# stripe/rainier

Hardware: AMD Instinct MI355X
Metric: leapfrog steps/sec (all chains) (higher is better)
Workload: dtype f64

## Files before the change

rainier_amd/csrc/device/rh_lane.hip.h:

```cpp
#if RH_NROWTARGETS > 0 && !RH_HAS_GATHER && !RH_BIGTH && !RH_BIGN && !RH_LK_LDS
#ifndef RH_LANE_W
#define RH_LANE_W 8
#endif
#ifndef RH_LANE_R
#define RH_LANE_R 8
#endif
#ifndef RH_LANE_C
#define RH_LANE_C 2
#endif
#ifndef RH_LANE_FEED_ROWS
#define RH_LANE_FEED_ROWS 0
#endif
typedef const double __attribute__((address_space(4))) *rh_ccol_t;
struct rh_lane_rows { const double *p[RH_NROWTARGETS]; };
constexpr bool rh_lane_rowfed(int nc) { return RH_LANE_FEED_ROWS && (nc == 1 || nc == 2 || nc == 4 || nc == 8); }
constexpr int rh_lane_set(int nc) { return 16 / nc < RH_LANE_R ? 16 / nc : RH_LANE_R; }
template <int S, int NC> RH_DEV void rh_lane_request(double (&c)[S][NC], rh_ccol_t rp, const long long row) {
#pragma unroll
  for (int u = 0; u < S; u++)
#pragma unroll
    for (int j = 0; j < NC; j++) c[u][j] = rp[(row + u) * NC + j];
}
template <int S, int NC> RH_DEV void rh_lane_arrived(const double (&c)[S][NC]) {
#pragma unroll
  for (int u = 0; u < S; u++)
#pragma unroll
    for (int j = 0; j < NC; j++) asm volatile("" ::"s"(c[u][j]));
}
template <int T, bool NV>
RH_DEV void rh_lane_targets(const double (&th)[RH_LANE_C][RH_NTH], const rh_model_data &d, const rh_lane_rows *rows, const int w, const int split, const int nsplit,
                            const int *__restrict__ lp, const int nvalid, const int chains, double *__restrict__ partial,
                            double *red, int &err) {
  if constexpr (T < RH_NTARGETS) {
    typedef rh_target<T> TG;
    if constexpr (TG::HAS_ROWS) {
      constexpr int NC = TG::NCOLS, R = RH_LANE_R, C = RH_LANE_C, W = RH_LANE_W;
      constexpr int NA = TG::NACC > 0 ? TG::NACC : 1;
      const int lane = threadIdx.x & 63;
      double inv[C][TG::NINV > 0 ? TG::NINV : 1];
#pragma unroll
      for (int k = 0; k < C; k++) TG::invariants(th[k], inv[k], err);
      const long long n = d.nrows[T];
      const long long blocks = (n + R - 1) / R, per = (blocks + nsplit - 1) / nsplit, perw = (per + W - 1) / W;
      long long s0 = (long long)split * per * R, s1 = s0 + per * R;
      if (s0 > n) s0 = n;
      if (s1 > n) s1 = n;
      long long r0 = s0 + (long long)w * perw * R, r1 = r0 + perw * R;
      if (r0 > s1) r0 = s1;
      if (r1 > s1) r1 = s1;
      rh_ccol_t cp[NC];
#pragma unroll
      for (int j = 0; j < NC; j++) cp[j] = (rh_ccol_t)d.cols[TG::COL0 + j];
      double acc[C][NA];
#pragma unroll
      for (int k = 0; k < C; k++)
#pragma unroll
        for (int o = 0; o < NA; o++) acc[k][o] = 0.0;
      long long kb = r0;
      if constexpr (rh_lane_rowfed(NC)) {
        constexpr int S = rh_lane_set(NC);
        static_assert(R % S == 0 && S * NC * 2 * 2 <= 64, "two sets of whole rows in 64 scalar registers, a block of R rows in whole sets");
        const rh_ccol_t rp = (rh_ccol_t)rows->p[TG::ROWT];
        const int nsets = (int)((r1 - kb) / S);
        const long long last = kb + (long long)(nsets > 0 ? nsets - 1 : 0) * S;
        auto rows_of = [&](const double (&cur)[S][NC]) {
#pragma unroll
          for (int u = 0; u < S; u++)
#pragma unroll
            for (int k = 0; k < C; k++) rh_row<TG, NV>(th[k], inv[k], cur[u], acc[k], err);
// ... 23 lines not shown
        double c[R][NC];
#pragma unroll
        for (int u = 0; u < R; u++)
#pragma unroll
          for (int j = 0; j < NC; j++) c[u][j] = cp[j][kb + u];
#pragma unroll
        for (int u = 0; u < R; u++)
#pragma unroll
          for (int k = 0; k < C; k++) rh_row<TG, NV>(th[k], inv[k], c[u], acc[k], err);
      }
      for (; kb < r1; kb++) {
        double c[NC];
#pragma unroll
        for (int j = 0; j < NC; j++) c[j] = cp[j][kb];
#pragma unroll
        for (int k = 0; k < C; k++) rh_row<TG, NV>(th[k], inv[k], c, acc[k], err);
      }
      }
#pragma unroll
      for (int k = 0; k < C; k++)
#pragma unroll
        for (int o = 0; o < NA; o++) red[((w * C + k) * NA + o) * 64 + lane] = acc[k][o];
      __syncthreads();
      for (int t = threadIdx.x; t < C * NA * 64; t += 64 * W) {
        const int ko = t >> 6, l = t & 63, k = ko / NA, o = ko - k * NA;
        double s = red[ko * 64 + l];
#pragma unroll
        for (int ww = 1; ww < W; ww++) s += red[(ww * C * NA + ko) * 64 + l];
        const int slot = k * 64 + l;
        if (slot < nvalid) partial[(((size_t)TG::ROWT * nsplit + split) * chains + lp[slot]) * RH_NACC_MAX + o] = s;
      }
      __syncthreads();
    }
    rh_lane_targets<T + 1, NV>(th, d, rows, w, split, nsplit, lp, nvalid, chains, partial, red, err);
  }
}
RH_DEV void rh_grad_lane_body(const rh_model_data &d, const rh_lane_rows *rows, const double *__restrict__ q, const int *__restrict__ list,
                              const int *__restrict__ nlive, const int *__restrict__ vflag, double *__restrict__ partial, int *__restrict__ err_out,
                              int *__restrict__ n_running, const int chains, const int nsplit, const int xcd_aware, double *red) {
  const int lane = threadIdx.x & 63, w = __builtin_amdgcn_readfirstlane((int)(threadIdx.x >> 6));
  const int b = blockIdx.x;
  if (b == 0 && threadIdx.x == 0) *n_running = 0;
  const int nl = rh_live_count(nlive, chains);
  int split, group;
  rh_grad_map(b, nsplit, xcd_aware, split, group);
  const int slot0 = group * (64 * RH_LANE_C);
  if (slot0 >= nl) return;
  double th[RH_LANE_C][RH_NTH];
  bool gonly = rh_any_value_only<0>::v && vflag != nullptr;
#pragma unroll
  for (int k = 0; k < RH_LANE_C; k++) {
    const int c = rh_live_chain(list, slot0 + k * 64 + lane, nl);
    if constexpr (rh_any_value_only<0>::v) gonly = gonly && vflag[c] == 2;
#pragma unroll
    for (int i = 0; i < RH_NVARS; i++) th[k][i] = q[(size_t)c * RH_NVARS + i];
  }
  int err = 0;
  if constexpr (rh_any_value_only<0>::v) {
    if (__all(gonly)) rh_lane_targets<0, false>(th, d, rows, w, split, nsplit, list + slot0, nl - slot0, chains, partial, red, err);
    else rh_lane_targets<0, true>(th, d, rows, w, split, nsplit, list + slot0, nl - slot0, chains, partial, red, err);
  } else
  rh_lane_targets<0, true>(th, d, rows, w, split, nsplit, list + slot0, nl - slot0, chains, partial, red, err);
  if (__any(err != 0) && lane == 0) atomicOr(err_out, 1);
}
#if !RH_LANE_FEED_ROWS
extern "C" __global__ void __launch_bounds__(64 * RH_LANE_W)
rh_grad_lane_kernel(const rh_model_data d, const double *__restrict__ q, const int *__restrict__ list, const int *__restrict__ nlive,
                    const int *__restrict__ vflag, double *__restrict__ partial, int *__restrict__ err_out, int *__restrict__ n_running,
                    const int chains, const int nsplit, const int xcd_aware) {
  __shared__ double red[RH_LANE_W * RH_LANE_C * RH_NACC_MAX * 64];
  rh_grad_lane_body(d, nullptr, q, list, nlive, vflag, partial, err_out, n_running, chains, nsplit, xcd_aware, red);
}
#else
extern "C" __global__ void __launch_bounds__(64 * RH_LANE_W)
rh_grad_lane_kernel(const rh_model_data d, const rh_lane_rows rows, const double *__restrict__ q, const int *__restrict__ list,
                    const int *__restrict__ nlive, const int *__restrict__ vflag, double *__restrict__ partial, int *__restrict__ err_out,
                    int *__restrict__ n_running, const int chains, const int nsplit, const int xcd_aware) {
  __shared__ double red[RH_LANE_W * RH_LANE_C * RH_NACC_MAX * 64];
  rh_grad_lane_body(d, &rows, q, list, nlive, vflag, partial, err_out, n_running, chains, nsplit, xcd_aware, red);
}
#endif
#endif
```

rainier_amd/csrc/engine.cpp:

```cpp
#include <hip/hip_runtime.h>
#include <hip/hiprtc.h>

#include <cmath>
#include <chrono>
#include <cstdio>
#include <cstdlib>
#include <cstring>
#include <algorithm>
#include <atomic>
#include <fstream>
#include <functional>
#include <map>
#include <memory>
#include <mutex>
#include <sstream>
#include <string>
#include <thread>
#include <vector>

#include <dlfcn.h>
#include <sys/stat.h>
#include <unistd.h>

#include "../../include/rainier_hip.h"
// ... 188 lines not shown
  bool pending = false, prev_rec = false;
  std::vector<int> livelog[2];
  std::vector<char> was_ticked[2];
};
struct RoundRec {
  bool open = false;
  int pool = 0;
  bool live[2] = {false, false};
  int B[2] = {0, 0};
};

struct rh_sampler {
  hipFunction_t k_chain = nullptr, k_tick = nullptr;
  int state_words = 0, dense_off = 0, pack_l = 64;
  int off_Pq = -1, off_Pg = -1, off_PU = -1;
  rh_model *m = nullptr;
  rh_cfg_dev cfg{};
  int chains = 0;
  void *d_state = nullptr, *d_seeds = nullptr, *d_mass = nullptr, *d_draws = nullptr, *d_stats = nullptr, *d_running = nullptr;
  int it_done = 0;
  bool started = false, warmed = false;
  hipEvent_t e0 = nullptr, e1 = nullptr;
  double kernel_ms = 0, total_ms = 0;
  int64_t chain_slots = 0, steady_launches = 0, steady_evals = 0;
  double steady_ms = 0;
  int64_t launches = 0;
  bool tick_engine = false;
  int nsplit = 0, xcd_aware = 1;
  bool compact = true;
  void *d_qbuf = nullptr, *d_active = nullptr;
  void *d_rec[2] = {nullptr, nullptr};
  bool fuse = false;
  bool lane_walk = false;
  bool lane_rows = false;
  std::vector<Lane> lanes;
  int round_cap = 0;
  int next_pool = 0;
  RoundRec round;
  std::vector<rh_chain_stats_dev> last_stats;
  int64_t grads_at_reset = 0;
};
int guard(rh_model *m, const std::function<void()> &fn) {
  try { fn(); return RH_OK; }
  catch (const Fail &f) { g_err = f.msg; if (m) m->err = f.msg; return f.code; }
  catch (const std::exception &e) { g_err = e.what(); if (m) m->err = e.what(); return RH_E_INVALID; }
}
DrawsView sampler_draws(rh_sampler *s) {
  return {s->d_draws, s->m->device, s->m->stream, s->chains, s->it_done, (int)s->m->prog.n_params, s->cfg.iterations, &s->m->mu, &s->m->err, s->m};
}

namespace {

void assemble_source(rh_model *m) {
  std::string defines, targets, err;
  if (const char *e = rh::knob("RH_GRAD_PIPELINE")) m->eopt.grad_pipeline = std::atoi(e);
  if (const char *e = rh::knob("RH_FMA_ADDS")) m->eopt.fma_adds = std::atoi(e) != 0;
  if (const char *e = rh::knob("RH_XFUSE")) m->eopt.xfuse = std::atoi(e) != 0;
  if (const char *e = rh::knob("RH_SIMPLIFY")) m->eopt.simplify = std::atoi(e) != 0;
  if (const char *e = rh::knob("RH_PACK")) m->eopt.pack = std::atoi(e) != 0;
  if (const char *e = rh::knob("RH_FAST_LOG")) m->eopt.fast_log = std::atoi(e) != 0;
  if (const char *e = rh::knob("RH_FORCE_BIGN")) m->eopt.force_bign = std::atoi(e) != 0;
  if (const char *e = rh::knob("RH_LOGIT_LINK")) m->eopt.logit_link = std::atoi(e) != 0;
  if (const char *e = rh::knob("RH_CONST_POOL")) m->eopt.const_pool = std::atoi(e) != 0;
  if (const char *e = rh::knob("RH_CHUNK")) if (m->eopt.chunk == 0) m->eopt.chunk = std::max(0, std::atoi(e));
  if (m->eopt.chunk > 0) {
    m->eopt.rows_unroll = 1; m->eopt.grad_unroll = 1; m->eopt.grad_pipeline = 0; m->unroll_auto = false;
    m->eopt.grad_chains = 1;
// ... 1219 lines not shown
        void *sb = nullptr;
        const size_t bytes = sizeof(double) * (size_t)chains * m->gather_count[rt];
        HIPCHK(hipMalloc(&sb, bytes));
        owned.push_back(sb);
        HIPCHK(hipMemset(sb, 0, bytes));
        gd.sbuf[rt] = (double *)sb;
      }
    }
    HIPCHK(hipDeviceSynchronize());
  }
  ~GatherBufs() { for (void *p : owned) (void)hipFree(p); }
};

int default_nsplit(const rh_model *m, int chains) {
  const int ngroups = (chains + m->grad_k - 1) / m->grad_k;
  int64_t max_rows = 1;
  for (size_t t = 0; t < m->prog.targets.size(); t++) if (m->prog.targets[t].n_cols) max_rows = std::max<int64_t>(max_rows, m->data.nrows[t]);
  int nsplit = (int)std::max<int64_t>(1, ((m->eopt.grad_pipeline == 2 ? 2048 : 4096) + ngroups - 1) / ngroups);
  if (m->info.gather_mode) nsplit = (int)std::max<int64_t>(1, (16384 + ngroups - 1) / ngroups);
  if (const char *e = rh::knob("RH_GATHER_WG")) if (m->info.gather_mode) nsplit = (int)std::max<int64_t>(1, (std::atoi(e) + ngroups - 1) / ngroups);
  if (m->k_grad_glm) { const int ctiles = (chains + 15) / 16; nsplit = (int)std::max<int64_t>(1, (2048 + ctiles - 1) / ctiles); }
  nsplit = ((nsplit + 7) / 8) * 8;
  const int64_t cap = std::max<int64_t>(8, (max_rows / 2048) / 8 * 8);
  return (int)std::min<int64_t>(nsplit, cap);
}

int64_t lane_max_rows(const rh_model *m) {
  int64_t max_rows = 1;
  for (size_t t = 0; t < m->prog.targets.size(); t++) if (m->prog.targets[t].n_cols) max_rows = std::max<int64_t>(max_rows, m->data.nrows[t]);
  return max_rows;
}
thread_local int g_total_chains = 0;
thread_local int g_shard_walk = -1;
bool walk_is_lane(rh_model *m, bool static_hmc, int total_chains) {
  if (g_shard_walk >= 0) return g_shard_walk == 1 && ensure_lane(m) != nullptr;
  int forced = 0;
  if (const char *e = rh::knob("RH_GRAD_WALK")) forced = std::strcmp(e, "tile") == 0 ? 1 : (std::strcmp(e, "lane") == 0 ? 2 : 0);
  if (!rh_plan::walk_is_lane(true, static_hmc, m->grad_chains_req, total_chains, lane_max_rows(m), forced)) return false;
  return ensure_lane(m) != nullptr;
}
int lane_nsplit(const rh_model *m, int total_chains) {
  return rh_plan::lane_nsplit(total_chains, lane_max_rows(m));
}
bool feed_is_rows(rh_model *m) {
  int forced = 0;
  if (const char *e = rh::knob("RH_LANE_FEED")) forced = std::strcmp(e, "cols") == 0 ? 1 : (std::strcmp(e, "rows") == 0 ? 2 : 0);
  if (!rh_plan::feed_is_rows(true, forced)) return false;
  if (!rh_plan::feed_is_rows(ensure_lane_rows(m) != nullptr, forced)) return false;
  std::vector<long long> want;
  for (size_t t = 0; t < m->prog.targets.size(); t++) if (m->prog.targets[t].n_cols) want.push_back(m->data.nrows[t]);
  return m->k_grad_lane_rows && rh_plan::lane_rows_cover((int)want.size(), want.data(), (int)m->dev_rows_n.size(), m->dev_rows_n.data(), m->dev_rows.data());
}

void launch_grad(rh_model *m, GatherBufs *gb, void *d_q, void *d_list, void *d_nlive, void *d_vflag, void *d_partial, void *d_graderr, void *d_running,
                 int chains, int nsplit, int xcd, hipStream_t stream = nullptr, bool lane_walk = false, bool lane_rows = false) {
  if (!stream) stream = m->stream;
  if (lane_walk) {
    const int lgroups = (chains + rh_plan::kLaneGroup - 1) / rh_plan::kLaneGroup;
    if (lane_rows) {
      void *ra[] = {&m->data, m->dev_rows.data(), &d_q, &d_list, &d_nlive, &d_vflag, &d_partial, &d_graderr, &d_running, &chains, &nsplit, &xcd};
      launch(m->k_grad_lane_rows, (unsigned)(lgroups * nsplit), 64 * rh_plan::kLaneW, stream, ra);
      return;
    }
    void *la[] = {&m->data, &d_q, &d_list, &d_nlive, &d_vflag, &d_partial, &d_graderr, &d_running, &chains, &nsplit, &xcd};
    launch(m->k_grad_lane, (unsigned)(lgroups * nsplit), 64 * rh_plan::kLaneW, stream, la);
    return;
  }
  const int ngroups = (chains + m->grad_k - 1) / m->grad_k;
  if (m->info.gather_mode) {
    void *ga[] = {&m->data, &gb->gd, &d_q, &d_list, &d_nlive, &d_vflag, &d_partial, &d_graderr, &d_running, &chains, &nsplit};
    if (gb->any_big) launch(m->k_grad_gather, (unsigned)(ngroups * nsplit), 64, stream, ga);
    if (gb->any_small) launch(m->k_grad_gather_scan, (unsigned)(ngroups * nsplit), 64, stream, ga);
    return;
  }
  void *args[] = {&m->data, &d_q, &d_list, &d_nlive, &d_vflag, &d_partial, &d_graderr, &d_running, &chains, &nsplit, &xcd};
  if (m->k_grad_glm) {
    const int ctiles = (chains + 15) / 16;
    const unsigned blocks = (unsigned)(((ctiles + m->glm_w - 1) / m->glm_w) * nsplit);
    const unsigned tile = (unsigned)m->glm_ncols * 66u * (unsigned)sizeof(double);
    const unsigned lds = (2u * tile + (m->lk_lds ? 6176u : 0u) <= 160u * 1024u ? 2u : 1u) * tile;
    HIPCHK(hipModuleLaunchKernel(m->k_grad_glm, blocks, 1, 1, 64u * m->glm_w, 1, 1, lds, stream, args, nullptr));
  } else
    launch(m->k_grad, (unsigned)(ngroups * nsplit), 64, stream, args);
}
}

extern "C" int rh_density_eval(rh_model *m, const double *q, int32_t chains, double *logp, double *grad) {
  return rh_density_eval_ex(m, q, chains, RH_ENGINE_AUTO, 0, logp, grad);
}

extern "C" int rh_density_eval_ex(rh_model *m, const double *q, int32_t chains, int32_t engine, int32_t grad_splits,
                                  double *logp, double *grad) {
  if (!m || !m->loaded) { g_err = "rh_density_eval: model not loaded"; return RH_E_INVALID; }
  if (!q || !logp || !grad || chains <= 0) { m->err = g_err = "rh_density_eval: bad arguments"; return RH_E_INVALID; }
  if (engine < RH_ENGINE_AUTO || engine > RH_ENGINE_TICK || grad_splits < 0 || grad_splits > 65536) { m->err = g_err = "rh_density_eval_ex: unknown engine / bad grad_splits"; return RH_E_INVALID; }
  if (engine == RH_ENGINE_TICK && m->n_row_targets == 0) { m->err = g_err = "the tick engine needs a model that streams rows"; return RH_E_INVALID; }
  if (engine == RH_ENGINE_CHAIN && m->info.gather_mode) { m->err = g_err = "gather-mode models run on the tick engine only"; return RH_E_UNSUPPORTED; }
  const bool use_tick = m->info.gather_mode || engine == RH_ENGINE_TICK || (engine == RH_ENGINE_AUTO && !m->density_ok && m->tick_ok);
  if (use_tick && !m->tick_ok) { m->err = g_err = "the tick engine's kernels of this model are not fit to run: " + m->tick_why; return RH_E_UNSUPPORTED; }
  if (!use_tick && !m->density_ok) { m->err = g_err = "rh_density_kernel of this model is not fit to run: " + m->density_why; return RH_E_UNSUPPORTED; }
  std::lock_guard<std::mutex> lk(m->mu);
  int lookup_err = 0;
  const int rc = guard(m, [&] {
    HIPCHK(hipSetDevice(m->device));
    const int n = (int)m->prog.n_params;
    DevBuf bq(sizeof(double) * n * chains), bl(sizeof(double) * chains), bg(sizeof(double) * n * chains), be(sizeof(int));
    const bool bigth = m->info.bign && !m->info.gather_mode && (n > 512 || m->eopt.chunk > 0);
    DevBuf btot(bigth ? sizeof(double) * (size_t)(n + 1) * chains : 8);
    void *dq = bq.p, *dl = bl.p, *dg = bg.p, *de = be.p, *dtot = btot.p;
    HIPCHK(hipMemcpyAsync(dq, q, sizeof(double) * n * chains, hipMemcpyHostToDevice, m->stream));
    HIPCHK(hipMemsetAsync(de, 0, sizeof(int), m->stream));
    int ch = chains;
    if (use_tick) {
      const bool lane_walk = walk_is_lane(m, false, chains);
      const bool lane_rows = lane_walk && feed_is_rows(m);
      int nsplit = grad_splits > 0 ? grad_splits : (m->info.gather_mode ? 64 : lane_walk ? lane_nsplit(m, chains) : default_nsplit(m, chains));
      GatherBufs gb;
      if (m->info.gather_mode) gb.build(m, chains, nsplit);
      const size_t pbytes = sizeof(double) * (size_t)m->n_row_targets * nsplit * chains * m->nacc_max;
      DevBuf bpart(pbytes), brun(sizeof(int)), blist(sizeof(int) * chains);
      { std::vector<int> ident((size_t)chains);
        for (int c = 0; c < chains; c++) ident[(size_t)c] = c;
        HIPCHK(hipMemcpyAsync(blist.p, ident.data(), sizeof(int) * chains, hipMemcpyHostToDevice, m->stream));
        HIPCHK(hipStreamSynchronize(m->stream)); }
      HIPCHK(hipMemsetAsync(bpart.p, 0, pbytes, m->stream));
      int xcd = 1;
      if (const char *e = rh::knob("RH_XCD_AWARE")) xcd = std::atoi(e);
      void *dnl = nullptr;
      std::unique_ptr<DevBuf> bnl;
      if (const char *e = rh::knob("RH_EVAL_LIVE")) {
        std::vector<int> live;
        for (const char *p = e; *p;) { char *q2; long v = std::strtol(p, &q2, 10); if (q2 == p) break; if (v >= 0 && v < chains) live.push_back((int)v); p = *q2 ? q2 + 1 : q2; }
        std::sort(live.begin(), live.end());
        live.erase(std::unique(live.begin(), live.end()), live.end());
        if (!live.empty()) {
          const int nl = (int)live.size();
          HIPCHK(hipMemcpyAsync(blist.p, live.data(), sizeof(int) * nl, hipMemcpyHostToDevice, m->stream));
          bnl.reset(new DevBuf(sizeof(int)));
          HIPCHK(hipMemcpyAsync(bnl->p, &nl, sizeof(int), hipMemcpyHostToDevice, m->stream));
          HIPCHK(hipStreamSynchronize(m->stream));
          dnl = bnl->p;
        }
      }
      launch_grad(m, &gb, dq, blist.p, dnl, nullptr, bpart.p, de, brun.p, chains, nsplit, xcd, nullptr, lane_walk, lane_rows);
      void *dpart = bpart.p;
      if (m->info.gather_mode) {
        void *fa[] = {&m->data, &gb.gd, &dq, &dpart, &dl, &dg, &de, &ch, &nsplit, &dtot};
        launch(m->k_density_fin, (unsigned)chains, 64, m->stream, fa);
      } else {
        void *fa[] = {&m->data, &dq, &dpart, &dl, &dg, &de, &ch, &nsplit, &dtot};
        launch(m->k_density_fin, (unsigned)chains, 64, m->stream, fa);
      }
      HIPCHK(hipMemcpyAsync(logp, dl, sizeof(double) * chains, hipMemcpyDeviceToHost, m->stream));
      HIPCHK(hipMemcpyAsync(grad, dg, sizeof(double) * n * chains, hipMemcpyDeviceToHost, m->stream));
      HIPCHK(hipMemcpyAsync(&lookup_err, de, sizeof(int), hipMemcpyDeviceToHost, m->stream));
      HIPCHK(hipStreamSynchronize(m->stream));
      return;
    }
    void *args[] = {&m->data, &dq, &dl, &dg, &de, &ch, &dtot};
    launch(m->k_density, (unsigned)((chains + 64 / m->info.pack_l - 1) / (64 / m->info.pack_l)), 64, m->stream, args);
    HIPCHK(hipMemcpyAsync(logp, dl, sizeof(double) * chains, hipMemcpyDeviceToHost, m->stream));
    HIPCHK(hipMemcpyAsync(grad, dg, sizeof(double) * n * chains, hipMemcpyDeviceToHost, m->stream));
    HIPCHK(hipMemcpyAsync(&lookup_err, de, sizeof(int), hipMemcpyDeviceToHost, m->stream));
    HIPCHK(hipStreamSynchronize(m->stream));
  });
  if (rc == RH_OK && lookup_err) { m->err = g_err = "Lookup index out of range during evaluation"; return RH_E_LOOKUP; }
  return rc;
}

extern "C" int rh_selftest(rh_model *m, int32_t mode, int64_t seed, const double *in, double *out, int32_t n) {
  if (!m || !m->loaded || !out || n <= 0) { g_err = "rh_selftest: bad arguments"; return RH_E_INVALID; }
  std::lock_guard<std::mutex> lk(m->mu);
  return guard(m, [&] {
    HIPCHK(hipSetDevice(m->device));
    const size_t in_n = (mode == 5 || mode == 14) ? 2 * (size_t)n : (size_t)n;
    DevBuf bin(sizeof(double) * in_n), bout(sizeof(double) * n);
    void *din = bin.p, *dout = bout.p;
// ... 132 lines not shown
    d.iterations = cfg->iterations; d.warmup = cfg->warmup; d.sampler = cfg->sampler; d.hmc_steps = cfg->hmc_steps;
    d.ehmc_max_steps = cfg->ehmc_max_steps; d.ehmc_min_steps = cfg->ehmc_min_steps; d.ehmc_buf_size = cfg->ehmc_buf_size;
    d.step_tuner = cfg->step_tuner; d.ehmc_p_count = cfg->ehmc_p_count; d.dualavg_delta = cfg->dualavg_delta;
    d.static_step = cfg->static_step; d.mass_tuner = cfg->mass_tuner; d.mass_init_window = cfg->mass_init_window;
    d.mass_skip_first = cfg->mass_skip_first; d.mass_skip_last = cfg->mass_skip_last; d.mass_expansion = cfg->mass_expansion;
    d.nuts_max_depth = cfg->nuts_max_depth;
    HIPCHK(hipSetDevice(m->device));
    const int n = (int)m->prog.n_params;
    const size_t state_bytes = (size_t)chains * s->state_words * sizeof(uint64_t);
    HIPCHK(hipMalloc(&s->d_state, state_bytes));
    HIPCHK(hipMalloc(&s->d_seeds, sizeof(int64_t) * 2 * chains));
    HIPCHK(hipMalloc(&s->d_mass, sizeof(double) * n));
    const size_t draws_bytes = (size_t)chains * (size_t)(cfg->iterations ? cfg->iterations : 1) * n * sizeof(double);
    HIPCHK(hipMalloc(&s->d_draws, draws_bytes));
    HIPCHK(hipMalloc(&s->d_stats, sizeof(rh_chain_stats_dev) * chains));
    HIPCHK(hipMalloc(&s->d_running, sizeof(int)));
    {
      std::vector<int64_t> rec((size_t)2 * chains);
      for (int c = 0; c < chains; c++) {
        const double nn = cfg->rng_next_gaussian ? cfg->rng_next_gaussian[c] : std::nan("");
        rec[2 * c] = seeds[c];
        std::memcpy(&rec[2 * c + 1], &nn, sizeof nn);
      }
      HIPCHK(hipMemcpy(s->d_seeds, rec.data(), sizeof(int64_t) * rec.size(), hipMemcpyHostToDevice));
    }
    std::vector<double> mass(n, 1.0);
    if (cfg->mass_tuner == RH_MASS_STATIC_DIAG) mass.assign(cfg->static_mass, cfg->static_mass + n);
    HIPCHK(hipMemcpy(s->d_mass, mass.data(), sizeof(double) * n, hipMemcpyHostToDevice));
    HIPCHK(hipMemset(s->d_draws, 0, draws_bytes));
    HIPCHK(hipEventCreate(&s->e0));
    HIPCHK(hipEventCreate(&s->e1));
    s->last_stats.resize(chains);
    if (s->tick_engine) {
      s->lane_walk = walk_is_lane(m, cfg->sampler == RH_SAMPLER_HMC, g_total_chains > 0 ? g_total_chains : chains);
      s->lane_rows = s->lane_walk && feed_is_rows(m);
      int nsplit = cfg->grad_splits;
      if (nsplit <= 0) nsplit = s->lane_walk ? lane_nsplit(m, g_total_chains > 0 ? g_total_chains : chains) : default_nsplit(m, chains);
      int subf = cfg->sampler == RH_SAMPLER_HMC ? 1 : 8;
      if (const char *e = rh::knob("RH_SUBF")) { subf = 1; while (subf * 2 <= std::atoi(e) && subf < 64) subf *= 2; }
      if (const char *e = rh::knob("RH_COMPACT")) s->compact = std::atoi(e) != 0;
      { int64_t max_rows = 1;
        for (size_t t = 0; t < m->prog.targets.size(); t++) if (m->prog.targets[t].n_cols) max_rows = std::max<int64_t>(max_rows, m->data.nrows[t]);
        while (subf > 1 && max_rows / ((int64_t)nsplit * subf) < 1024) subf >>= 1; }
      if (!m->k_compact) s->compact = false;
      nsplit *= subf;
      if (nsplit > 65536) throw Fail{RH_E_INVALID, "grad_splits too large"};
      s->nsplit = nsplit;
      if (const char *e = rh::knob("RH_XCD_AWARE")) s->xcd_aware = std::atoi(e);
      HIPCHK(hipMalloc(&s->d_qbuf, sizeof(double) * n * chains));
      HIPCHK(hipMalloc(&s->d_active, sizeof(int) * chains));
      HIPCHK(hipMemset(s->d_qbuf, 0, sizeof(double) * n * chains));
      HIPCHK(hipMemset(s->d_active, 0, sizeof(int) * chains));
      const size_t rec_u64 = (size_t)(3 * n + 8);
      {
        bool fuse = m->k_grad_fused && m->k_absorb && s->k_tick == m->k_tick && cfg->sampler == RH_SAMPLER_HMC && !m->k_grad_glm && !s->lane_walk;
        if (const char *e = rh::knob("RH_FUSE")) fuse = fuse && std::atoi(e) != 0;
        if (fuse) {
          const size_t rec_bytes = sizeof(uint64_t) * rec_u64 * chains;
          for (int k = 0; k < 2; k++) { HIPCHK(hipMalloc(&s->d_rec[k], rec_bytes)); HIPCHK(hipMemset(s->d_rec[k], 0, rec_bytes)); }
          s->fuse = true;
        }
      }
      int forced = 0;
      if (const char *e = rh::knob("RH_LANES")) forced = std::atoi(e) == 1 ? 1 : (std::atoi(e) == 2 ? 2 : 0);
      const rh_plan::LaneCut cut = rh_plan::lanes_cut(chains, s->lane_walk ? rh_plan::kLaneGroup : m->k_grad_glm ? 16 : m->grad_k, nsplit,
                                                      s->lane_walk ? rh_plan::kLaneW : m->k_grad_glm ? m->glm_w : 1, device_cus(m->device), forced);
      s->lanes.resize((size_t)cut.lanes);
      s->round_cap = rh_plan::kRoundCapDefault;
      if (const char *e = rh::knob("RH_ROUND_MAX")) s->round_cap = rh_plan::round_cap(std::atoi(e));
      const size_t cap = (size_t)s->round_cap;
      const size_t iters_alloc = (size_t)cfg->iterations;
// ... 57 lines not shown
    for (int li = 0; li < nl; li++) {
      if (!R.live[li]) continue;
      Lane &L = s->lanes[(size_t)li];
      float a = 0, b = 0;
      if (!ref) ref = L.r0[p]; else HIPCHK(hipEventElapsedTime(&a, ref, L.r0[p]));
      HIPCHK(hipEventElapsedTime(&b, L.r0[p], L.r1[p]));
      t0[k] = a; t1[k] = (double)a + b; k++;
    }
    s->total_ms += k == 1 ? t1[0] - t0[0] : rh_plan::busy_shares(k, t0, t1, share);
  }
  std::vector<double> t0, t1, share;
  for (int li = 0; li < nl; li++) {
    if (!R.live[li]) continue;
    Lane &L = s->lanes[(size_t)li];
    for (int i = 0; i < R.B[li]; i++) {
      float a = 0, g = 0;
      if (nlive > 1) HIPCHK(hipEventElapsedTime(&a, ref, L.ev[p][(size_t)2 * i]));
      HIPCHK(hipEventElapsedTime(&g, L.ev[p][(size_t)2 * i], L.ev[p][(size_t)2 * i + 1]));
      t0.push_back(a); t1.push_back((double)a + g);
    }
  }
  share.resize(t0.size());
  if (nlive > 1) rh_plan::busy_shares((int)t0.size(), t0.data(), t1.data(), share.data());
  else for (size_t i = 0; i < t0.size(); i++) share[i] = t1[i] - t0[i];
  size_t at = 0;
  for (int li = 0; li < nl; li++) {
    if (!R.live[li]) continue;
    Lane &L = s->lanes[(size_t)li];
    for (int i = 0; i < R.B[li]; i++, at++) {
      const double g = share[at];
      s->kernel_ms += g;
      const int served = L.cur_live;
      s->chain_slots += served;
      if ((int64_t)served * 10 >= (int64_t)L.chains * 9) { s->steady_ms += g; s->steady_launches += 1; s->steady_evals += served; }
      if (s->compact && L.was_ticked[p][(size_t)i]) L.cur_live = L.livelog[p][(size_t)i];
    }
    s->launches += R.B[li];
  }
}
}

extern "C" void rh_sampler_destroy(rh_sampler *s) {
  if (!s) return;
  if (s->m) hipSetDevice(s->m->device);
  if (s->m) (void)guard(nullptr, [&] { resolve_round(s); });
  for (void *p : {s->d_state, s->d_seeds, s->d_mass, s->d_draws, s->d_stats, s->d_running, s->d_qbuf, s->d_active, s->d_rec[0], s->d_rec[1]})
    if (p) hipFree(p);
  for (Lane &L : s->lanes) {
    for (void *p : {L.d_running, L.d_list, L.d_nlive, L.d_livelog, L.d_partial, L.d_partial2, L.d_graderr})
      if (p) hipFree(p);
    for (int p = 0; p < 2; p++) {
      for (hipEvent_t e : L.ev[p]) hipEventDestroy(e);
      if (L.r0[p]) hipEventDestroy(L.r0[p]);
      if (L.r1[p]) hipEventDestroy(L.r1[p]);
    }
    if (L.e0) hipEventDestroy(L.e0);
    if (L.e1) hipEventDestroy(L.e1);
    delete L.gb;
    if (L.own_stream && L.stream) hipStreamDestroy(L.stream);
  }
  if (s->e0) hipEventDestroy(s->e0);
  if (s->e1) hipEventDestroy(s->e1);
  delete s;
}

namespace {
void advance_to_ticks(rh_sampler *s, int it_stop) {
  rh_model *m = s->m;
  HIPCHK(hipSetDevice(m->device));
  resolve_round(s);
  int nsplit = s->nsplit, stop = it_stop, xcd = s->xcd_aware;
  void *no_list = nullptr;
  bool value_free = true;
  if (const char *e = rh::knob("RH_VALUE_FREE")) if (std::atoi(e) == 0) value_free = false;
  auto tick = [&](Lane &L, int fresh, bool reset_counter, void *partial, bool listed, int log_slot) {
    int chains = L.chains;
    if (reset_counter) HIPCHK(hipMemsetAsync(L.d_running, 0, sizeof(int), L.stream));
    void *lst = listed && s->compact ? L.d_list : no_list, *nl = listed && s->compact ? L.d_nlive : no_list;
    if (m->info.gather_mode) {
      void *args[] = {&m->data, &L.gb->gd, &s->cfg, &L.state, &L.seeds, &s->d_mass, &L.draws, &L.stats, &L.d_running, &L.qbuf,
                      &L.active, &partial, &L.d_graderr, &lst, &nl, &chains, &nsplit, &stop, &fresh};
      launch(s->k_tick, (unsigned)chains, 64, L.stream, args);
    } else {
      void *args[] = {&m->data, &s->cfg, &L.state, &L.seeds, &s->d_mass, &L.draws, &L.stats, &L.d_running, &L.qbuf,
                      &L.active, &partial, &L.d_graderr, &lst, &nl, &chains, &nsplit, &stop, &fresh};
      launch(s->k_tick, (unsigned)chains, 64, L.stream, args);
    }
    if (s->compact) {
      void *lg = (int *)L.d_livelog + log_slot;
      void *ca[] = {&L.active, &L.d_list, &L.d_nlive, &lg, &chains};
      launch(m->k_compact, 1u, 1024, L.stream, ca);
    }
  };
  auto grad = [&](Lane &L, void *partial) {
    launch_grad(m, L.gb, L.qbuf, L.d_list, s->compact ? L.d_nlive : nullptr ,
                value_free ? L.active : nullptr, partial, L.d_graderr, L.d_running, L.chains, nsplit, xcd, L.stream, s->lane_walk, s->lane_rows);
  };
  auto grad_fused = [&](Lane &L, void *partial_in, void *partial_out, void *rec_in, void *rec_out) {
    int chains = L.chains;
    void *live_n = s->compact ? L.d_nlive : nullptr;
    void *args[] = {&m->data, &L.qbuf, &L.d_list, &live_n, &partial_in, &partial_out, &L.d_graderr, &L.d_running, &L.state, &rec_in, &rec_out,
                    &chains, &nsplit, &xcd};
    launch(m->k_grad_fused, (unsigned)(((chains + m->grad_k - 1) / m->grad_k) * nsplit), 64, L.stream, args);
  };
  auto absorb = [&](Lane &L, void *rec) {
    int chains = L.chains;
    void *args[] = {&L.state, &rec, &L.qbuf, &L.active, &chains};
    launch(m->k_absorb, (unsigned)chains, 64, L.stream, args);
  };
  const int Ltraj = std::max(1, s->cfg.hmc_steps);
  const bool fuse_now = s->fuse && s->warmed && s->cfg.sampler == RH_SAMPLER_HMC && Ltraj > 1;
  const bool lock_step = s->cfg.sampler == RH_SAMPLER_HMC && s->warmed;
  const long long todo = lock_step ? (long long)std::max(0, it_stop - (s->cfg.warmup + s->it_done)) * Ltraj : 0;
  auto add_total = [&]() {
    hipEvent_t ref = nullptr;
    double t0[2], t1[2], share[2];
    int k = 0;
    for (Lane &L : s->lanes) {
      if (!L.live) continue;
      float a = 0, b = 0;
      if (!ref) ref = L.e0; else HIPCHK(hipEventElapsedTime(&a, ref, L.e0));
      HIPCHK(hipEventElapsedTime(&b, L.e0, L.e1));
      t0[k] = a; t1[k] = (double)a + b; k++;
    }
    s->total_ms += k == 1 ? t1[0] - t0[0] : rh_plan::busy_shares(k, t0, t1, share);
  };
  for (Lane &L : s->lanes) {
    L.live = true; L.pos = 0; L.remaining = todo;
    HIPCHK(hipEventRecord(L.e0, L.stream));
// ... 226 lines not shown
  if (!s || !s->m) return RH_E_INVALID;
  if (device) *device = s->m->device;
  if (stream) *stream = (void *)s->m->stream;
  if (doubles) *doubles = (int64_t)s->chains * (int64_t)s->cfg.iterations * (int64_t)s->m->prog.n_params;
  return RH_OK;
}
extern "C" void rh_set_thread_error_(const char *msg) { g_err = msg ? msg : ""; }

extern "C" int rh_sampler_lane_feed(const rh_sampler *s) {
  if (!s) { g_err = "rh_sampler_lane_feed: NULL"; return -RH_E_INVALID; }
  return !s->lane_walk ? 0 : (s->lane_rows ? 2 : 1);
}
extern "C" int rh_sampler_progress(const rh_sampler *s, int32_t *warmed, int32_t *iterations_done) {
  if (!s) { g_err = "rh_sampler_progress: NULL"; return RH_E_INVALID; }
  if (warmed) *warmed = s->warmed ? 1 : 0;
  if (iterations_done) *iterations_done = s->it_done;
  return RH_OK;
}
extern "C" int rh_sampler_timing(rh_sampler *s, rh_timing *out, int reset) {
  if (!s || !out) { g_err = "rh_sampler_timing: NULL"; return RH_E_INVALID; }
  std::lock_guard<std::mutex> lk(s->m->mu);
  return guard(s->m, [&] {
    fetch_stats(s);
    resolve_round(s);
    int64_t grads = 0;
    for (auto &d : s->last_stats) grads += d.gradient_evaluations;
    std::memset(out, 0, sizeof(*out));
    out->kernel_ms = s->kernel_ms; out->total_ms = s->total_ms; out->launches = s->launches;
    out->density_evals = grads - s->grads_at_reset;
    out->row_chain_evals = out->density_evals * s->m->rows_total;
    std::snprintf(out->dominant_kernel, sizeof out->dominant_kernel, s->tick_engine ? (s->m->info.gather_mode ? "rh_grad_gather_kernel" : s->m->k_grad_glm ? "rh_grad_glm_kernel" : s->lane_walk ? "rh_grad_lane_kernel" : (s->fuse && s->warmed && s->cfg.hmc_steps > 1) ? "rh_grad_fused_kernel" : "rh_grad_kernel") : "rh_chain_kernel");
    out->chain_slots = s->tick_engine ? s->chain_slots : out->density_evals;
    out->steady_kernel_ms = s->steady_ms; out->steady_launches = s->steady_launches; out->steady_density_evals = s->steady_evals;
    if (reset) { s->kernel_ms = 0; s->total_ms = 0; s->launches = 0; s->grads_at_reset = grads; s->chain_slots = 0; s->steady_ms = 0; s->steady_launches = 0; s->steady_evals = 0; }
  });
}

extern "C" int rh_sample(rh_model *m, const rh_config *cfg, const int64_t *seeds, int32_t chains, double *draws,
                         double *mass_diag, rh_chain_stats *stats) {
  rh_sampler *s = nullptr;
  int rc = rh_sampler_create(m, cfg, seeds, chains, &s);
  if (rc != RH_OK) return rc;
  rc = rh_sampler_warmup(s);
  if (rc == RH_OK) rc = rh_sampler_run(s, cfg->iterations);
  if (rc == RH_OK && draws && cfg->iterations > 0) rc = rh_sampler_draws(s, 0, cfg->iterations, draws);
  if (rc == RH_OK) rc = rh_sampler_stats(s, stats, mass_diag);
  rh_sampler_destroy(s);
  return rc;
}

extern "C" int rh_sample_multi(rh_model *const *models, int32_t n_models, const rh_config *cfg, const int64_t *seeds,
                               int32_t chains, double *draws, double *mass_diag, rh_chain_stats *stats) {
  if (!models || n_models <= 0 || !cfg || !seeds || chains <= 0) { g_err = "rh_sample_multi: bad arguments"; return RH_E_INVALID; }
  if (cfg->struct_size != (int32_t)sizeof(rh_config)) { g_err = "rh_config.struct_size mismatch"; return RH_E_INVALID; }
  const int nv = models[0] ? rh_model_nvars(models[0]) : -1;
  for (int g = 0; g < n_models; g++) {
    if (!models[g] || !models[g]->loaded) { g_err = "rh_sample_multi: model " + std::to_string(g) + " not loaded"; return RH_E_INVALID; }
    if (rh_model_nvars(models[g]) != nv) { g_err = "rh_sample_multi: the models differ (nvars)"; return RH_E_INVALID; }
  }
  const int G = std::min<int>(n_models, chains);
  int splits_all = cfg->grad_splits;
  bool lane_all = models[0]->n_row_targets > 0;
  for (int g = 0; g < G && lane_all; g++) lane_all = walk_is_lane(models[g], cfg->sampler == RH_SAMPLER_HMC, chains);
  if (splits_all <= 0 && models[0]->n_row_targets > 0) splits_all = lane_all ? lane_nsplit(models[0], chains) : default_nsplit(models[0], chains);
  std::vector<int> first((size_t)G + 1, 0);
  for (int g = 0; g < G; g++) first[(size_t)g + 1] = first[(size_t)g] + chains / G + (g < chains % G ? 1 : 0);
  std::vector<int> rcs((size_t)G, RH_OK);
  std::vector<std::string> errs((size_t)G);
  std::vector<std::thread> th;
  for (int g = 0; g < G; g++)
    th.emplace_back([&, g] {
      const int c0 = first[(size_t)g], nc = first[(size_t)g + 1] - c0;
      rh_config c = *cfg;
      c.grad_splits = splits_all;
      if (cfg->rng_next_gaussian) c.rng_next_gaussian = cfg->rng_next_gaussian + c0;
      const size_t per_chain = (size_t)cfg->iterations * (size_t)nv;
      g_total_chains = chains; g_shard_walk = lane_all ? 1 : 0;
      rcs[(size_t)g] = rh_sample(models[g], &c, seeds + c0, nc, draws ? draws + (size_t)c0 * per_chain : nullptr,
                                 mass_diag ? mass_diag + (size_t)c0 * nv : nullptr, stats ? stats + c0 : nullptr);
      g_total_chains = 0; g_shard_walk = -1;
      if (rcs[(size_t)g] != RH_OK) errs[(size_t)g] = rh_last_error(models[g]);
    });
  for (auto &t : th) t.join();
  for (int g = 0; g < G; g++)
    if (rcs[(size_t)g] != RH_OK) { g_err = "shard " + std::to_string(g) + ": " + errs[(size_t)g]; return rcs[(size_t)g]; }
  return RH_OK;
}
```

rainier_amd/csrc/lanes_plan.hpp:

```cpp
#ifndef RH_LANES_PLAN_HPP
#define RH_LANES_PLAN_HPP

#include <algorithm>
#include <vector>

namespace rh_plan {
struct LaneCut { int lanes, first[2], count[2]; };
inline LaneCut lanes_cut(int chains, int group, int nsplit, int waves_per_wg, int cus, int forced) {
  LaneCut one = {1, {0, 0}, {chains, 0}};
  const int ngroups = (chains + group - 1) / group;
  if (forced == 1 || ngroups < 2) return one;
  const int cg = std::max(1, std::min(ngroups - 1, (chains + group) / (2 * group)));
  const int cut = cg * group;
  const long long smaller = std::min(cg, ngroups - cg);
  if (forced != 2 && smaller * nsplit * waves_per_wg < 4LL * cus) return one;
  return {2, {0, cut}, {cut, chains - cut}};
}

constexpr int kLaneW = 8, kLaneR = 8, kLaneC = 2, kLaneGroup = 64 * kLaneC;
constexpr int kLaneMinChains = 512;
constexpr long long kLaneMinEvals = 512LL * 1000000LL;
inline bool lane_walk_fits_r(int ncols_max, int nacc_max, int r) {
  return ncols_max >= 1 && ncols_max * r * 2 <= 64 && nacc_max >= 1 && (long long)kLaneW * kLaneC * nacc_max * 64 * 8 <= 64 * 1024;
}
inline bool lane_walk_fits(int ncols_max, int nacc_max) { return lane_walk_fits_r(ncols_max, nacc_max, kLaneR); }
inline bool walk_is_lane(bool model_has_lane, bool static_hmc, int grad_chains, int total_chains, long long max_rows, int forced) {
  if (!model_has_lane || forced == 1) return false;
  if (forced == 2) return true;
  return static_hmc && grad_chains == 0 && total_chains >= kLaneMinChains && (long long)total_chains * max_rows >= kLaneMinEvals;
}
inline int lane_nsplit(int total_chains, long long max_rows) {
  const long long ngroups = std::max(1, (total_chains + kLaneGroup - 1) / kLaneGroup);
  long long nsplit = std::max<long long>(1, (8192 + ngroups * kLaneW - 1) / (ngroups * kLaneW));
  nsplit = ((nsplit + 7) / 8) * 8;
  const long long cap = std::max<long long>(8, (max_rows / 512) / 8 * 8);
  return (int)std::min(nsplit, cap);
}

inline int lane_rows_set(int nc, int r = kLaneR) { return nc >= 1 && nc <= 16 ? std::min(r, 16 / nc) : 0; }
inline bool lane_rows_eligible(int nc, int r = kLaneR) {
  if (!(nc == 1 || nc == 2 || nc == 4 || nc == 8)) return false;
  const int set = lane_rows_set(nc, r);
  return set >= 1 && 2 * set * nc * 2 <= 64 && r % set == 0 && 8 % set == 0;
}
inline long long lane_rows_padded(long long rows) { return (rows + 7) / 8 * 8; }
inline long long lane_rows_doubles(long long rows, int nc) { return lane_rows_padded(rows) * nc; }
inline long long lane_rows_index(long long r, int nc, int j) { return r * nc + j; }
inline void lane_rows_place_column(const double *col, long long rows, int nc, int j, double *out) {
  for (long long r = 0; r < rows; r++) out[lane_rows_index(r, nc, j)] = col[r];
}
inline void lane_rows_interleave(const double *const *cols, long long rows, int nc, double *out) {
  for (int j = 0; j < nc; j++) lane_rows_place_column(cols[j], rows, nc, j, out);
  for (long long i = rows * nc, e = lane_rows_doubles(rows, nc); i < e; i++) out[i] = 0.0;
}
inline bool lane_rows_cover(int n_want, const long long *want, int n_have, const long long *have, const void *const *copy) {
  if (n_want != n_have) return false;
  for (int i = 0; i < n_want; i++) if (copy[i] && want[i] > have[i]) return false;
  return true;
}
constexpr bool kLaneFeedRowsDefault = true;
inline bool feed_is_rows(bool model_has_rows_kernel, int forced) {
  if (!model_has_rows_kernel || forced == 1) return false;
  return forced == 2 || kLaneFeedRowsDefault;
}

constexpr int kRoundCapDefault = 4096, kRoundMaxDynamic = 256, kRoundHint = 32;
inline int round_cap(int requested) { return std::max(1, std::min(requested, kRoundCapDefault)); }
inline int round_launches(bool lock_step, long long remaining, int ltraj, int cap) {
  const long long c = std::max(1, cap);
// ... 31 lines not shown
```

Baseline: 3.802 million.

## Run lane gradient groups with a single chain column when only one wavefront is live

Templates the lane gradient targets on the per-lane chain count and adds a path where a group with at most 64 live chains evaluates only one chain column instead of RH_LANE_C. This avoids spending row-processing work on padded, dead chain slots in the tail group, at the cost of an extra template instantiation and higher code size. It also adds a sampler-kind enum so dynamic samplers (eHMC/NUTS) explicitly stay off the lane walk by default, plus a lane split-factor helper and an optional live-count log file.

```diff
diff --git a/rainier_amd/csrc/device/rh_lane.hip.h b/rainier_amd/csrc/device/rh_lane.hip.h
--- a/rainier_amd/csrc/device/rh_lane.hip.h
+++ b/rainier_amd/csrc/device/rh_lane.hip.h
@@ -11,6 +11,7 @@
 #ifndef RH_LANE_FEED_ROWS
 #define RH_LANE_FEED_ROWS 0
 #endif
+#define RH_LANE_HALF_PATH (RH_LANE_FEED_ROWS && RH_LANE_C > 1 && !rh_any_value_only<0>::v)
 typedef const double __attribute__((address_space(4))) *rh_ccol_t;
 struct rh_lane_rows { const double *p[RH_NROWTARGETS]; };
 constexpr bool rh_lane_rowfed(int nc) { return RH_LANE_FEED_ROWS && (nc == 1 || nc == 2 || nc == 4 || nc == 8); }
@@ -27,14 +28,14 @@
 #pragma unroll
     for (int j = 0; j < NC; j++) asm volatile("" ::"s"(c[u][j]));
 }
-template <int T, bool NV>
-RH_DEV void rh_lane_targets(const double (&th)[RH_LANE_C][RH_NTH], const rh_model_data &d, const rh_lane_rows *rows, const int w, const int split, const int nsplit,
+template <int T, bool NV, int C>
+RH_DEV void rh_lane_targets(const double (&th)[C][RH_NTH], const rh_model_data &d, const rh_lane_rows *rows, const int w, const int split, const int nsplit,
                             const int *__restrict__ lp, const int nvalid, const int chains, double *__restrict__ partial,
                             double *red, int &err) {
   if constexpr (T < RH_NTARGETS) {
     typedef rh_target<T> TG;
     if constexpr (TG::HAS_ROWS) {
-      constexpr int NC = TG::NCOLS, R = RH_LANE_R, C = RH_LANE_C, W = RH_LANE_W;
+      constexpr int NC = TG::NCOLS, R = RH_LANE_R, W = RH_LANE_W;
       constexpr int NA = TG::NACC > 0 ? TG::NACC : 1;
       const int lane = threadIdx.x & 63;
       double inv[C][TG::NINV > 0 ? TG::NINV : 1];
@@ -124,13 +125,35 @@
       }
       __syncthreads();
     }
-    rh_lane_targets<T + 1, NV>(th, d, rows, w, split, nsplit, lp, nvalid, chains, partial, red, err);
+    rh_lane_targets<T + 1, NV, C>(th, d, rows, w, split, nsplit, lp, nvalid, chains, partial, red, err);
   }
+}
+template <int C>
+RH_DEV void rh_lane_group(const rh_model_data &d, const rh_lane_rows *rows, const double *__restrict__ q, const int *__restrict__ list,
+                          const int *__restrict__ vflag, double *__restrict__ partial, int *__restrict__ err_out, const int chains, const int nsplit,
+                          const int w, const int split, const int slot0, const int nl, double *red) {
+  const int lane = threadIdx.x & 63;
+  double th[C][RH_NTH];
+  bool gonly = rh_any_value_only<0>::v && vflag != nullptr;
+#pragma unroll
+  for (int k = 0; k < C; k++) {
+    const int c = rh_live_chain(list, slot0 + k * 64 + lane, nl);
+    if constexpr (rh_any_value_only<0>::v) gonly = gonly && vflag[c] == 2;
+#pragma unroll
+    for (int i = 0; i < RH_NVARS; i++) th[k][i] = q[(size_t)c * RH_NVARS + i];
+  }
+  int err = 0;
+  if constexpr (rh_any_value_only<0>::v) {
+    if (__all(gonly)) rh_lane_targets<0, false, C>(th, d, rows, w, split, nsplit, list + slot0, nl - slot0, chains, partial, red, err);
+    else rh_lane_targets<0, true, C>(th, d, rows, w, split, nsplit, list + slot0, nl - slot0, chains, partial, red, err);
+  } else
+  rh_lane_targets<0, true, C>(th, d, rows, w, split, nsplit, list + slot0, nl - slot0, chains, partial, red, err);
+  if (__any(err != 0) && lane == 0) atomicOr(err_out, 1);
 }
 RH_DEV void rh_grad_lane_body(const rh_model_data &d, const rh_lane_rows *rows, const double *__restrict__ q, const int *__restrict__ list,
                               const int *__restrict__ nlive, const int *__restrict__ vflag, double *__restrict__ partial, int *__restrict__ err_out,
-                              int *__restrict__ n_running, const int chains, const int nsplit, const int xcd_aware, double *red) {
-  const int lane = threadIdx.x & 63, w = __builtin_amdgcn_readfirstlane((int)(threadIdx.x >> 6));
+                              int *__restrict__ n_running, const int chains, const int nsplit, const int xcd_aware, const int half, double *red) {
+  const int w = __builtin_amdgcn_readfirstlane((int)(threadIdx.x >> 6));
   const int b = blockIdx.x;
   if (b == 0 && threadIdx.x == 0) *n_running = 0;
   const int nl = rh_live_count(nlive, chains);
@@ -138,38 +161,29 @@
   rh_grad_map(b, nsplit, xcd_aware, split, group);
   const int slot0 = group * (64 * RH_LANE_C);
   if (slot0 >= nl) return;
-  double th[RH_LANE_C][RH_NTH];
-  bool gonly = rh_any_value_only<0>::v && vflag != nullptr;
-#pragma unroll
-  for (int k = 0; k < RH_LANE_C; k++) {
-    const int c = rh_live_chain(list, slot0 + k * 64 + lane, nl);
-    if constexpr (rh_any_value_only<0>::v) gonly = gonly && vflag[c] == 2;
-#pragma unroll
-    for (int i = 0; i < RH_NVARS; i++) th[k][i] = q[(size_t)c * RH_NVARS + i];
+  if constexpr (RH_LANE_HALF_PATH) {
+    if (half != 0 && nl - slot0 <= 64) {
+      rh_lane_group<1>(d, rows, q, list, vflag, partial, err_out, chains, nsplit, w, split, slot0, nl, red);
+      return;
+    }
   }
-  int err = 0;
-  if constexpr (rh_any_value_only<0>::v) {
-    if (__all(gonly)) rh_lane_targets<0, false>(th, d, rows, w, split, nsplit, list + slot0, nl - slot0, chains, partial, red, err);
-    else rh_lane_targets<0, true>(th, d, rows, w, split, nsplit, list + slot0, nl - slot0, chains, partial, red, err);
-  } else
-  rh_lane_targets<0, true>(th, d, rows, w, split, nsplit, list + slot0, nl - slot0, chains, partial, red, err);
-  if (__any(err != 0) && lane == 0) atomicOr(err_out, 1);
+  rh_lane_group<RH_LANE_C>(d, rows, q, list, vflag, partial, err_out, chains, nsplit, w, split, slot0, nl, red);
 }
 #if !RH_LANE_FEED_ROWS
 extern "C" __global__ void __launch_bounds__(64 * RH_LANE_W)
 rh_grad_lane_kernel(const rh_model_data d, const double *__restrict__ q, const int *__restrict__ list, const int *__restrict__ nlive,
                     const int *__restrict__ vflag, double *__restrict__ partial, int *__restrict__ err_out, int *__restrict__ n_running,
-                    const int chains, const int nsplit, const int xcd_aware) {
+                    const int chains, const int nsplit, const int xcd_aware, const int half) {
   __shared__ double red[RH_LANE_W * RH_LANE_C * RH_NACC_MAX * 64];
-  rh_grad_lane_body(d, nullptr, q, list, nlive, vflag, partial, err_out, n_running, chains, nsplit, xcd_aware, red);
+  rh_grad_lane_body(d, nullptr, q, list, nlive, vflag, partial, err_out, n_running, chains, nsplit, xcd_aware, half, red);
 }
 #else
 extern "C" __global__ void __launch_bounds__(64 * RH_LANE_W)
 rh_grad_lane_kernel(const rh_model_data d, const rh_lane_rows rows, const double *__restrict__ q, const int *__restrict__ list,
                     const int *__restrict__ nlive, const int *__restrict__ vflag, double *__restrict__ partial, int *__restrict__ err_out,
-                    int *__restrict__ n_running, const int chains, const int nsplit, const int xcd_aware) {
+                    int *__restrict__ n_running, const int chains, const int nsplit, const int xcd_aware, const int half) {
   __shared__ double red[RH_LANE_W * RH_LANE_C * RH_NACC_MAX * 64];
-  rh_grad_lane_body(d, &rows, q, list, nlive, vflag, partial, err_out, n_running, chains, nsplit, xcd_aware, red);
+  rh_grad_lane_body(d, &rows, q, list, nlive, vflag, partial, err_out, n_running, chains, nsplit, xcd_aware, half, red);
 }
 #endif
 #endif
diff --git a/rainier_amd/csrc/engine.cpp b/rainier_amd/csrc/engine.cpp
--- a/rainier_amd/csrc/engine.cpp
+++ b/rainier_amd/csrc/engine.cpp
@@ -244,7 +244,9 @@
   void *d_rec[2] = {nullptr, nullptr};
   bool fuse = false;
   bool lane_walk = false;
+  int lane_half = 1;
   bool lane_rows = false;
+  FILE *live_fp = nullptr;
   std::vector<Lane> lanes;
   int round_cap = 0;
   int next_pool = 0;
@@ -1530,11 +1532,14 @@
 }
 thread_local int g_total_chains = 0;
 thread_local int g_shard_walk = -1;
-bool walk_is_lane(rh_model *m, bool static_hmc, int total_chains) {
+rh_plan::LaneSampler lane_sampler(int sampler) {
+  return sampler == RH_SAMPLER_HMC ? rh_plan::LaneSampler::StaticHmc : (sampler == RH_SAMPLER_NUTS ? rh_plan::LaneSampler::Nuts : rh_plan::LaneSampler::Ehmc);
+}
+bool walk_is_lane(rh_model *m, rh_plan::LaneSampler kind, int total_chains) {
   if (g_shard_walk >= 0) return g_shard_walk == 1 && ensure_lane(m) != nullptr;
   int forced = 0;
   if (const char *e = rh::knob("RH_GRAD_WALK")) forced = std::strcmp(e, "tile") == 0 ? 1 : (std::strcmp(e, "lane") == 0 ? 2 : 0);
-  if (!rh_plan::walk_is_lane(true, static_hmc, m->grad_chains_req, total_chains, lane_max_rows(m), forced)) return false;
+  if (!rh_plan::walk_is_lane(true, kind, m->grad_chains_req, total_chains, lane_max_rows(m), forced)) return false;
   return ensure_lane(m) != nullptr;
 }
 int lane_nsplit(const rh_model *m, int total_chains) {
@@ -1550,17 +1555,22 @@
   return m->k_grad_lane_rows && rh_plan::lane_rows_cover((int)want.size(), want.data(), (int)m->dev_rows_n.size(), m->dev_rows_n.data(), m->dev_rows.data());
 }
 
+int lane_half_on() {
+  if (const char *e = rh::knob("RH_LANE_HALF")) return std::atoi(e) != 0 ? 1 : 0;
+  return 1;
+}
+
 void launch_grad(rh_model *m, GatherBufs *gb, void *d_q, void *d_list, void *d_nlive, void *d_vflag, void *d_partial, void *d_graderr, void *d_running,
-                 int chains, int nsplit, int xcd, hipStream_t stream = nullptr, bool lane_walk = false, bool lane_rows = false) {
+                 int chains, int nsplit, int xcd, hipStream_t stream = nullptr, bool lane_walk = false, bool lane_rows = false, int lane_half = 1) {
   if (!stream) stream = m->stream;
   if (lane_walk) {
     const int lgroups = (chains + rh_plan::kLaneGroup - 1) / rh_plan::kLaneGroup;
     if (lane_rows) {
-      void *ra[] = {&m->data, m->dev_rows.data(), &d_q, &d_list, &d_nlive, &d_vflag, &d_partial, &d_graderr, &d_running, &chains, &nsplit, &xcd};
+      void *ra[] = {&m->data, m->dev_rows.data(), &d_q, &d_list, &d_nlive, &d_vflag, &d_partial, &d_graderr, &d_running, &chains, &nsplit, &xcd, &lane_half};
       launch(m->k_grad_lane_rows, (unsigned)(lgroups * nsplit), 64 * rh_plan::kLaneW, stream, ra);
       return;
     }
-    void *la[] = {&m->data, &d_q, &d_list, &d_nlive, &d_vflag, &d_partial, &d_graderr, &d_running, &chains, &nsplit, &xcd};
+    void *la[] = {&m->data, &d_q, &d_list, &d_nlive, &d_vflag, &d_partial, &d_graderr, &d_running, &chains, &nsplit, &xcd, &lane_half};
     launch(m->k_grad_lane, (unsigned)(lgroups * nsplit), 64 * rh_plan::kLaneW, stream, la);
     return;
   }
@@ -1610,7 +1620,7 @@
     HIPCHK(hipMemsetAsync(de, 0, sizeof(int), m->stream));
     int ch = chains;
     if (use_tick) {
-      const bool lane_walk = walk_is_lane(m, false, chains);
+      const bool lane_walk = rh::knob("RH_GRAD_WALK") && walk_is_lane(m, rh_plan::LaneSampler::Ehmc, chains);
       const bool lane_rows = lane_walk && feed_is_rows(m);
       int nsplit = grad_splits > 0 ? grad_splits : (m->info.gather_mode ? 64 : lane_walk ? lane_nsplit(m, chains) : default_nsplit(m, chains));
       GatherBufs gb;
@@ -1640,7 +1650,7 @@
           dnl = bnl->p;
         }
       }
-      launch_grad(m, &gb, dq, blist.p, dnl, nullptr, bpart.p, de, brun.p, chains, nsplit, xcd, nullptr, lane_walk, lane_rows);
+      launch_grad(m, &gb, dq, blist.p, dnl, nullptr, bpart.p, de, brun.p, chains, nsplit, xcd, nullptr, lane_walk, lane_rows, lane_half_on());
       void *dpart = bpart.p;
       if (m->info.gather_mode) {
         void *fa[] = {&m->data, &gb.gd, &dq, &dpart, &dl, &dg, &de, &ch, &nsplit, &dtot};
@@ -1839,11 +1849,13 @@
     HIPCHK(hipEventCreate(&s->e1));
     s->last_stats.resize(chains);
     if (s->tick_engine) {
-      s->lane_walk = walk_is_lane(m, cfg->sampler == RH_SAMPLER_HMC, g_total_chains > 0 ? g_total_chains : chains);
+      s->lane_walk = walk_is_lane(m, lane_sampler(cfg->sampler), g_total_chains > 0 ? g_total_chains : chains);
       s->lane_rows = s->lane_walk && feed_is_rows(m);
+      s->lane_half = lane_half_on();
+      if (const char *e = rh::knob("RH_LIVE_LOG")) s->live_fp = std::fopen(e, "a");
       int nsplit = cfg->grad_splits;
       if (nsplit <= 0) nsplit = s->lane_walk ? lane_nsplit(m, g_total_chains > 0 ? g_total_chains : chains) : default_nsplit(m, chains);
-      int subf = cfg->sampler == RH_SAMPLER_HMC ? 1 : 8;
+      int subf = rh_plan::split_factor(s->lane_walk, cfg->sampler == RH_SAMPLER_HMC);
       if (const char *e = rh::knob("RH_SUBF")) { subf = 1; while (subf * 2 <= std::atoi(e) && subf < 64) subf *= 2; }
       if (const char *e = rh::knob("RH_COMPACT")) s->compact = std::atoi(e) != 0;
       { int64_t max_rows = 1;
@@ -1967,6 +1979,7 @@
       s->kernel_ms += g;
       const int served = L.cur_live;
       s->chain_slots += served;
+      if (s->live_fp) std::fprintf(s->live_fp, "%d %d\n", li, served);
       if ((int64_t)served * 10 >= (int64_t)L.chains * 9) { s->steady_ms += g; s->steady_launches += 1; s->steady_evals += served; }
       if (s->compact && L.was_ticked[p][(size_t)i]) L.cur_live = L.livelog[p][(size_t)i];
     }
@@ -1996,6 +2009,7 @@
   }
   if (s->e0) hipEventDestroy(s->e0);
   if (s->e1) hipEventDestroy(s->e1);
+  if (s->live_fp) std::fclose(s->live_fp);
   delete s;
 }
 
@@ -2029,7 +2043,7 @@
   };
   auto grad = [&](Lane &L, void *partial) {
     launch_grad(m, L.gb, L.qbuf, L.d_list, s->compact ? L.d_nlive : nullptr ,
-                value_free ? L.active : nullptr, partial, L.d_graderr, L.d_running, L.chains, nsplit, xcd, L.stream, s->lane_walk, s->lane_rows);
+                value_free ? L.active : nullptr, partial, L.d_graderr, L.d_running, L.chains, nsplit, xcd, L.stream, s->lane_walk, s->lane_rows, s->lane_half);
   };
   auto grad_fused = [&](Lane &L, void *partial_in, void *partial_out, void *rec_in, void *rec_out) {
     int chains = L.chains;
@@ -2322,7 +2336,8 @@
     std::snprintf(out->dominant_kernel, sizeof out->dominant_kernel, s->tick_engine ? (s->m->info.gather_mode ? "rh_grad_gather_kernel" : s->m->k_grad_glm ? "rh_grad_glm_kernel" : s->lane_walk ? "rh_grad_lane_kernel" : (s->fuse && s->warmed && s->cfg.hmc_steps > 1) ? "rh_grad_fused_kernel" : "rh_grad_kernel") : "rh_chain_kernel");
     out->chain_slots = s->tick_engine ? s->chain_slots : out->density_evals;
     out->steady_kernel_ms = s->steady_ms; out->steady_launches = s->steady_launches; out->steady_density_evals = s->steady_evals;
-    if (reset) { s->kernel_ms = 0; s->total_ms = 0; s->launches = 0; s->grads_at_reset = grads; s->chain_slots = 0; s->steady_ms = 0; s->steady_launches = 0; s->steady_evals = 0; }
+    if (reset) { s->kernel_ms = 0; s->total_ms = 0; s->launches = 0; s->grads_at_reset = grads; s->chain_slots = 0; s->steady_ms = 0; s->steady_launches = 0; s->steady_evals = 0;
+                 if (s->live_fp) std::fprintf(s->live_fp, "# reset\n"); }
   });
 }
 
@@ -2351,7 +2366,7 @@
   const int G = std::min<int>(n_models, chains);
   int splits_all = cfg->grad_splits;
   bool lane_all = models[0]->n_row_targets > 0;
-  for (int g = 0; g < G && lane_all; g++) lane_all = walk_is_lane(models[g], cfg->sampler == RH_SAMPLER_HMC, chains);
+  for (int g = 0; g < G && lane_all; g++) lane_all = walk_is_lane(models[g], lane_sampler(cfg->sampler), chains);
   if (splits_all <= 0 && models[0]->n_row_targets > 0) splits_all = lane_all ? lane_nsplit(models[0], chains) : default_nsplit(models[0], chains);
   std::vector<int> first((size_t)G + 1, 0);
   for (int g = 0; g < G; g++) first[(size_t)g + 1] = first[(size_t)g] + chains / G + (g < chains % G ? 1 : 0);
diff --git a/rainier_amd/csrc/lanes_plan.hpp b/rainier_amd/csrc/lanes_plan.hpp
--- a/rainier_amd/csrc/lanes_plan.hpp
+++ b/rainier_amd/csrc/lanes_plan.hpp
@@ -29,12 +29,28 @@
   if (forced == 2) return true;
   return static_hmc && grad_chains == 0 && total_chains >= kLaneMinChains && (long long)total_chains * max_rows >= kLaneMinEvals;
 }
+enum class LaneSampler { StaticHmc = 0, Ehmc = 1, Nuts = 2 };
+constexpr bool kLaneDynamicEhmc = false;
+constexpr bool kLaneDynamicNuts = false;
+inline bool walk_is_lane(bool model_has_lane, LaneSampler kind, int grad_chains, int total_chains, long long max_rows, int forced) {
+  if (kind == LaneSampler::StaticHmc) return walk_is_lane(model_has_lane, true, grad_chains, total_chains, max_rows, forced);
+  const bool on = kind == LaneSampler::Ehmc ? kLaneDynamicEhmc : (kind == LaneSampler::Nuts && kLaneDynamicNuts);
+  return walk_is_lane(model_has_lane, on, grad_chains, total_chains, max_rows, forced);
+}
 inline int lane_nsplit(int total_chains, long long max_rows) {
   const long long ngroups = std::max(1, (total_chains + kLaneGroup - 1) / kLaneGroup);
   long long nsplit = std::max<long long>(1, (8192 + ngroups * kLaneW - 1) / (ngroups * kLaneW));
   nsplit = ((nsplit + 7) / 8) * 8;
   const long long cap = std::max<long long>(8, (max_rows / 512) / 8 * 8);
   return (int)std::min(nsplit, cap);
+}
+inline int lane_subf() { return 1; }
+inline int split_factor(bool lane_walk, bool static_hmc) { return lane_walk ? lane_subf() : (static_hmc ? 1 : 8); }
+inline bool lane_half_group(int live) { return live >= 1 && live <= kLaneGroup / kLaneC; }
+inline long long lane_computed_slots(int live, bool half) {
+  if (live <= 0) return 0;
+  const int full = live / kLaneGroup, rest = live - full * kLaneGroup;
+  return (long long)full * kLaneGroup + (rest == 0 ? 0 : (half && lane_half_group(rest) ? kLaneGroup / kLaneC : kLaneGroup));
 }
 
 inline int lane_rows_set(int nc, int r = kLaneR) { return nc >= 1 && nc <= 16 ? std::min(r, 16 / nc) : 0; }
```

Result: no change. 3.779 million (-0.6%).
